# argumentcomputer/multi-stark

Measured on AMD Instinct MI355X. Metric: prove_trace_rows_per_sec, higher is better.
Workload: dtype u64; 1 GPU; U32-add + byte-table lookup (benches/multi_stark.rs), 2^20 additions per proof, bench_config(): log_blowup 2, 100 queries, 10+10 PoW bits, GoldilocksBlake3Config; witness (traces + claims, 64-bit words) in pinned host memory at step start: upload, from_stage_1 on the device and read-back inside the timed region; the library narrows byte-valued traces on host threads INSIDE the step before they cro; rows_per_proof=1048832, proof_bytes=1100053, parallelism=single GPU

## Files before the change

multi-stark_amd/csrc/lookup.hip:

```cpp
#include "lookup_params.h"
#include "msamd.h"
#include "program.h"

namespace msamd {

namespace {

constexpr int INV_CHUNK = 16;
constexpr int CLAIMS_CHUNK = 16;
__device__ __forceinline__ E2 message(const u64* __restrict__ a, u32 n, E2 beta, E2 gamma, const GammaPows& gp) {
  if (n <= gp.n) {
    GlAcc a0, a1;
    acc_init(a0);
    acc_init(a1);
    for (u32 k = 0; k < n; k++) {
      const u64 v = a[k];
      acc_mad(a0, v, gp.g[k].c0);
      acc_mad(a1, v, gp.g[k].c1);
    }
    return e2(gl_add(acc_reduce(a0), beta.c0), gl_add(acc_reduce(a1), beta.c1));
  }
  E2 f = e2(0);
  for (u32 k = n; k-- > 0;) {
    f = e2_mul(f, gamma);
// ... 110 lines not shown
    }
    E2 c = carry;
    if (i < nb) tot[i] = e2_add(c, e2_sub(sh[threadIdx.x], v));
    __syncthreads();
    if (threadIdx.x == 255) carry = e2_add(c, sh[255]);
    __syncthreads();
  }
  if (threadIdx.x == 0) *total = carry;
}
__global__ __launch_bounds__(256) void scan_add_k(E2* __restrict__ out, size_t n, const E2* __restrict__ block_prefix) {
  size_t base = (blockIdx.x * size_t(256) + threadIdx.x) * SCAN_ITEMS;
  E2 p = block_prefix[blockIdx.x];
#pragma unroll
  for (int k = 0; k < SCAN_ITEMS; k++)
    if (base + k < n) out[base + k] = e2_add(out[base + k], p);
}

__global__ __launch_bounds__(256) void claims_acc_k(const u64* __restrict__ data, const u64* __restrict__ offs, size_t n,
                                                    const ChallengeBG* __restrict__ ch, E2* __restrict__ partial) {
  __shared__ E2 sh[256];
  const E2 beta = ch->beta, gamma = ch->gamma;
  const GammaPows& gp = ch->gp;
  const size_t base = blockIdx.x * size_t(256 * CLAIMS_CHUNK) + threadIdx.x;
  E2 msg[CLAIMS_CHUNK];
  E2 sum = e2(0);
  int cnt = 0;
#pragma unroll
  for (int t = 0; t < CLAIMS_CHUNK; t++) {
    size_t i = base + size_t(t) * 256;
    if (i < n) {
// ... 84 lines not shown
  DBuf<E2> block_prefix;
  scan_exclusive(ctx, rowsum.p, prefix.p, n, total_dev, &block_prefix);
  ev = ctx.prof_begin(K_STAGE2);
  hipLaunchKernelGGL(stage2_write_k, grid, dim3(256), 0, ctx.stream, (const E2*)terms.p, n, logn, L, (const E2*)prefix.p, out,
                     (const E2*)block_prefix.p, SCAN_PER_BLOCK);
  ctx.prof_end(K_STAGE2, ev, double(n) * 16.0 * L);
  HIP_CHECK(hipGetLastError());
}

void stage2_from_trace_async(Ctx& ctx, const JitKernel& trace_jit, const u64* d_trace, const u64* d_pre, size_t n, size_t num_lookups,
                             size_t args_width, E2 beta, E2 gamma, u64* out, E2* total_dev) {
  DBuf<ChallengeBG> ch = challenge_bg_upload(ctx, beta, gamma);
  stage2_from_trace_dyn(ctx, trace_jit, d_trace, d_pre, n, num_lookups, args_width, ch.p, out, total_dev);
}
void stage2_from_trace_dyn(Ctx& ctx, const JitKernel& trace_jit, const u64* d_trace, const u64* d_pre, size_t n, size_t num_lookups,
                           size_t args_width, const ChallengeBG* ch, u64* out, E2* total_dev) {
  if (!trace_jit.function || num_lookups == 0) throw std::runtime_error("stage2_from_trace: no fused kernel for this circuit");
  const unsigned logn = log2_strict(n);
  const u32 L = (u32)num_lookups;
  DBuf<E2> rowsum(ctx, n), prefix(ctx, n), terms(ctx, n * L);
  dim3 grid((unsigned)((n + 255) / 256));
  Stage2TraceParams sp;
  sp.trace = d_trace;
  sp.pre = d_pre;
  sp.n = n;
  sp.ch = ch;
  sp.terms = terms.p;
  sp.rowsum = rowsum.p;
  hipEvent_t ev = ctx.prof_begin(K_STAGE2);
  stage2_trace_jit_launch(ctx, trace_jit, sp);
  ctx.prof_end(K_STAGE2, ev, double(n) * 8.0 * (L + args_width));
  DBuf<E2> block_prefix;
  scan_exclusive(ctx, rowsum.p, prefix.p, n, total_dev, &block_prefix);
  ev = ctx.prof_begin(K_STAGE2);
  hipLaunchKernelGGL(stage2_write_k, grid, dim3(256), 0, ctx.stream, (const E2*)terms.p, n, logn, L, (const E2*)prefix.p, out,
                     (const E2*)block_prefix.p, SCAN_PER_BLOCK);
  ctx.prof_end(K_STAGE2, ev, double(n) * 16.0 * L);
  HIP_CHECK(hipGetLastError());
}

E2 stage2_build(Ctx& ctx, const DLookups& lk, E2 beta, E2 gamma, u64* out, const JitKernel* jit) {
  DBuf<E2> tot(ctx, 1);
  stage2_build_async(ctx, lk, beta, gamma, out, tot.p, jit);
// ... 46 lines not shown
```

multi-stark_amd/csrc/lookup_params.h:

```cpp
#pragma once
#include "gl_dev.h"

namespace msamd {

constexpr int MAX_GPOW = 64;

struct GammaPows {
  E2 g[MAX_GPOW];
  u32 n;
};

struct ChallengeBG {
  E2 beta, gamma;
  GammaPows gp;
};
GL_HD void challenge_bg_fill(ChallengeBG& c, E2 beta, E2 gamma) {
  c.beta = beta;
  c.gamma = gamma;
  c.gp.n = MAX_GPOW;
  E2 g = e2(1);
  for (int i = 0; i < MAX_GPOW; i++) {
    c.gp.g[i] = g;
    g = e2_mul(g, gamma);
  }
// ... 3 lines not shown
  const u64* mult;
  const u64* args;
  size_t n;
  const ChallengeBG* ch;
  E2* terms;
  E2* rowsum;
};

struct Stage2TraceParams {
  const u64* trace;
  const u64* pre;
  size_t n;
  const ChallengeBG* ch;
  E2* terms;
  E2* rowsum;
};

}
```

multi-stark_amd/csrc/msamd.h:

```cpp
#pragma once
#include <hip/hip_runtime.h>

#include <cstdint>
#include <cstring>
#include <map>
#include <mutex>
#include <stdexcept>
#include <string>
#include <vector>

#include "gl_dev.h"

namespace msamd {

#define HIP_CHECK(expr)                                                                                   \
  do {                                                                                                    \
    hipError_t _e = (expr);                                                                               \
    if (_e != hipSuccess)                                                                                 \
      throw std::runtime_error(std::string("HIP error: ") + hipGetErrorString(_e) + " at " + __FILE__ + ":" + \
                               std::to_string(__LINE__));                                                 \
  } while (0)

static constexpr unsigned TW_LOG = 28;
static constexpr unsigned TW_HALF = 14;
// ... 172 lines not shown
  ~DBuf() { reset(); }
};

struct DMat {
  DBuf<u64> buf;
  size_t h = 0, w = 0;
  u64* d() const { return buf.p; }
};

struct NttSrc {
  const u64* src = nullptr;
  unsigned src_div = 1;
  const u64* scale = nullptr;
};
void ntt_dif(Ctx& ctx, u64* data, unsigned logn, size_t ncols, bool inverse, const NttSrc* from = nullptr, u64 out_mul = 1);
void ntt_dit(Ctx& ctx, u64* data, unsigned logn, size_t ncols, bool inverse, u64 out_mul = 1);
void transpose_in(Ctx& ctx, const u64* rowmajor, u64* colmajor, size_t h, size_t w, bool bitrev_rows);
void transpose_out(Ctx& ctx, const u64* colmajor, u64* rowmajor, size_t h, size_t w, bool bitrev_rows);
void pull_widen_words(const uint8_t* host_packed, unsigned bytes, size_t count, u64* out, hipStream_t stream);
void lde_from_coeffs(Ctx& ctx, const u64* coef, u64* lde, unsigned logn, unsigned log_blowup, size_t w);
void coset_lde(Ctx& ctx, u64* evals_bitrev, u64* lde, unsigned logn, unsigned log_blowup, size_t w);
void quotient_lde(Ctx& ctx, u64* qvals_bitrev, u64* lde, unsigned logn, unsigned logq, unsigned log_blowup, size_t D);

struct MatRef {
  const u64* d;
  uint32_t w;
  uint32_t pad;
  uint64_t stride;
};
struct DTree {
  std::vector<const u64*> mat_d;
  std::vector<size_t> mat_h, mat_w;
  std::vector<size_t> mat_stride;
  DBuf<Digest> digests;
  Digest* ext = nullptr;
  Digest* base() const { return ext ? ext : digests.p; }
// ... 34 lines not shown
                               u32* d_state12 = nullptr);

struct JitKernel;
struct DLookups {
  size_t height = 0, num_lookups = 0, args_width = 0;
  DBuf<u64> mult, args;
  DBuf<uint32_t> arg_offsets;
};
E2 stage2_build(Ctx& ctx, const DLookups& lk, E2 beta, E2 gamma, u64* out_colmajor_bitrev, const JitKernel* jit = nullptr);
void stage2_build_async(Ctx& ctx, const DLookups& lk, E2 beta, E2 gamma, u64* out_colmajor_bitrev, E2* total_dev,
                        const JitKernel* jit = nullptr);
struct ChallengeBG;
DBuf<ChallengeBG> challenge_bg_upload(Ctx& ctx, E2 beta, E2 gamma);
void stage2_build_dyn(Ctx& ctx, const DLookups& lk, const ChallengeBG* ch, u64* out_colmajor_bitrev, E2* total_dev, const JitKernel* jit = nullptr);
void stage2_from_trace_dyn(Ctx& ctx, const JitKernel& trace_jit, const u64* d_trace, const u64* d_pre, size_t n, size_t num_lookups,
                           size_t args_width, const ChallengeBG* ch, u64* out_colmajor_bitrev, E2* total_dev);
void claims_accumulator_dyn(Ctx& ctx, const u64* d_claim_data, const u64* d_claim_offsets, size_t n_claims, const ChallengeBG* ch, E2* out_dev);
void stage2_from_trace_async(Ctx& ctx, const JitKernel& trace_jit, const u64* d_trace, const u64* d_pre, size_t n, size_t num_lookups,
                             size_t args_width, E2 beta, E2 gamma, u64* out_colmajor_bitrev, E2* total_dev);
void claims_accumulator_async(Ctx& ctx, const u64* d_claim_data, const u64* d_claim_offsets, size_t n_claims, E2 beta, E2 gamma,
                              E2* out_dev);
E2 claims_accumulator(Ctx& ctx, const u64* d_claim_data, const u64* d_claim_offsets, size_t n_claims, E2 beta, E2 gamma);
size_t claims_transcript_words(Ctx& ctx, const u64* d_claim_data, const u64* d_claim_offsets, size_t n_claims,
                               size_t total_elems, u64* d_words);

void claims_transcript_words_slice(Ctx& ctx, const u64* d_data_abs, const u64* d_offs_first, size_t first, size_t count, size_t n_total,
                                   u64* d_words_abs);

struct JitKernel {
  void* module = nullptr;
  void* function = nullptr;
  bool inline_tables = false;
  unsigned groups = 0;
  JitKernel() {}
  JitKernel(const JitKernel&) = delete;
  JitKernel& operator=(const JitKernel&) = delete;
  JitKernel(JitKernel&& o) noexcept : module(o.module), function(o.function), inline_tables(o.inline_tables), groups(o.groups) {
    o.module = o.function = nullptr;
  }
  JitKernel& operator=(JitKernel&& o) noexcept {
    std::swap(module, o.module);
    std::swap(function, o.function);
    std::swap(inline_tables, o.inline_tables);
    std::swap(groups, o.groups);
    return *this;
  }
  ~JitKernel();
};
struct DProgram {
  JitKernel jit;
  DBuf<uint32_t> code;
  DBuf<u64> consts;
  size_t n_instr = 0, n_slots = 0;
  DBuf<uint32_t> zero_slots;
  DBuf<uint32_t> lookup_slots;
  size_t n_zeros = 0, n_lookups = 0, constraint_count = 0;
  size_t main_w = 0, pre_w = 0, s2_w = 0;
// ... 126 lines not shown
```

multi-stark_amd/csrc/ntt.hip:

```cpp
#include <cstring>

#include "msamd.h"

namespace msamd {

namespace {

__device__ __forceinline__ u64 tw_lookup(const u64* __restrict__ t0, const u64* __restrict__ t1, u32 e26) {
  return gl_mul(t1[e26 >> TW_HALF], t0[e26 & ((1u << TW_HALF) - 1)]);
}

template <int DIT>
__device__ __forceinline__ void lds_stages(u64* sm, unsigned k, unsigned logT, const u64* __restrict__ t1) {
  if (k == 0) return;
  const unsigned T = 1u << logT;
  const unsigned nb = (1u << (k - 1)) << logT;
  for (unsigned s = 0; s < k; s++) {
    const unsigned loghalf = DIT ? s : (k - 1 - s);
    const unsigned half = 1u << loghalf;
    const unsigned tsh = TW_HALF - loghalf - 1;
    for (unsigned b = threadIdx.x; b < nb; b += blockDim.x) {
      unsigned l = b & (T - 1), bb = b >> logT;
      unsigned j = bb & (half - 1), grp = bb >> loghalf;
      unsigned i0 = (((grp << (loghalf + 1)) + j) << logT) + l;
// ... 4 lines not shown
        u64 t = gl_mul(w, y);
        sm[i0] = gl_add(x, t);
        sm[i1] = gl_sub(x, t);
      } else {
        sm[i0] = gl_add(x, y);
        sm[i1] = gl_mul(gl_sub(x, y), w);
      }
    }
    __syncthreads();
  }
}

template <int DIT>
__global__ __launch_bounds__(256) void ntt_contig_k(const u64* __restrict__ src, u64* __restrict__ dst, unsigned K,
                                                     unsigned logn, const u64* __restrict__ t1, unsigned src_div,
                                                     const u64* __restrict__ scale, u64 out_mul) {
  extern __shared__ u64 sm[];
  const size_t n = size_t(1) << logn;
  const size_t col = blockIdx.y, off = size_t(blockIdx.x) << K;
  const u64* s = src + (col / src_div) * n + off;
  const u64* sc = scale ? scale + (col % src_div) * n + off : nullptr;
  u64* d = dst + col * n + off;
  const unsigned m = 1u << K;
  for (unsigned i = threadIdx.x; i < m; i += blockDim.x) {
    u64 v = s[i];
    if (sc) v = gl_mul(v, sc[i]);
    sm[i] = v;
  }
  __syncthreads();
  lds_stages<DIT>(sm, K, 0, t1);
  for (unsigned i = threadIdx.x; i < m; i += blockDim.x) {
    u64 v = sm[i];
    if (out_mul != 1) v = gl_mul(v, out_mul);
    d[i] = v;
  }
}

template <int DIT>
__global__ __launch_bounds__(256) void ntt_strided_k(const u64* __restrict__ src, u64* __restrict__ dst, unsigned k,
                                                      unsigned logS, unsigned logT, unsigned logn,
// ... 165 lines not shown
__device__ __forceinline__ void reg_round16(u64 (&x)[16], u32 lo, unsigned shift, const u64* __restrict__ twc, const u64* __restrict__ twx) {
#if MSAMD_R16TW
  (void)twc;
  reg_stages16_tw<DIT, INV>(x, lo, shift, twx);
#else
  reg_stages16_r4<DIT, INV>(x, lo, shift, twc, twx);
#endif
}

__device__ __forceinline__ u32 pad_hi(u32 e) { return e + ((e >> 8) << 4); }
__device__ __forceinline__ u32 pad_lo(u32 e) { return e + (e >> 4); }
constexpr int NTT12_LDS = 4096 + 256 + 16;
__device__ __forceinline__ u32 pad_half(u32 e) { return e + ((e >> 7) << 3); }
constexpr int NTT8S_LDS = 2048 + 128 + 8;

template <bool DIT, bool INV>
__global__ __launch_bounds__(256) void ntt12_k(const u64* __restrict__ src, u64* __restrict__ dst, unsigned logn,
                                               const u64* __restrict__ twc, const u64* __restrict__ twc3, unsigned src_div,
                                               const u64* __restrict__ scale, u64 out_mul) {
  __shared__ u64 sm[NTT12_LDS];
  const size_t n = size_t(1) << logn;
  const size_t col = blockIdx.y, off = size_t(blockIdx.x) << 12;
  const u64* s = src + (col / src_div) * n + off;
  const u64* sc = scale ? scale + (col % src_div) * n + off : nullptr;
  u64* d = dst + col * n + off;
  const u32 t = threadIdx.x, a = t >> 4, b = t & 15;
  u64 x[16];
#pragma unroll
  for (int j = 0; j < 16; j++) {
    u64 v = s[t + 256 * j];
    if (sc) v = gl_mul(v, sc[t + 256 * j]);
    x[j] = v;
  }
  if (!DIT) {
    reg_round16<false, INV>(x, t, 8, twc, twc3);
#pragma unroll
    for (int j = 0; j < 16; j++) sm[pad_hi(t + 256 * j)] = x[j];
    __syncthreads();
#pragma unroll
    for (int j = 0; j < 16; j++) x[j] = sm[pad_hi(a * 256 + 16 * j + b)];
    reg_round16<false, INV>(x, b, 4, twc, twc3);
    __syncthreads();
#pragma unroll
    for (int j = 0; j < 16; j++) sm[pad_lo(a * 256 + 16 * j + b)] = x[j];
    __syncthreads();
// ... 302 lines not shown
  unsigned logT = 12 - k;
  if (logT > logS) logT = logS;
  size_t gx = (size_t(1) << (logS - logT)) << (logn - logB);
  if (ncols > 65535) throw std::runtime_error("ntt: more than 65535 columns in one generic strided pass");
  dim3 grid((unsigned)gx, (unsigned)ncols);
  size_t shmem = (size_t(8) << (k + logT));
  hipEvent_t ev = ctx.prof_begin(K_NTT_STRIDED);
  hipLaunchKernelGGL(ntt_strided_k<DIT>, grid, dim3(256), shmem, ctx.stream, src, dst, k, logS, logT, logn,
                     inverse ? ctx.tw0i : ctx.tw0, inverse ? ctx.tw1i : ctx.tw1, src_div, scale, out_mul);
  HIP_CHECK(hipGetLastError());
  ctx.prof_end(K_NTT_STRIDED, ev, 16.0 * double(ncols) * double(size_t(1) << logn));
}

template <int DIT>
void launch_contig(Ctx& ctx, const u64* src, u64* dst, unsigned K, unsigned logn, size_t ncols, bool inverse,
                   unsigned src_div, const u64* scale, u64 out_mul) {
  dim3 grid((unsigned)(size_t(1) << (logn - K)), (unsigned)ncols);
  if (K == 12) {
    const int id = DIT ? K_NTT12_DIT : K_NTT12_DIF;
    hipEvent_t ev12 = ctx.prof_begin(id);
    if (inverse)
      hipLaunchKernelGGL((ntt12_k<(DIT != 0), true>), grid, dim3(256), 0, ctx.stream, src, dst, logn, ctx.twci, MSAMD_R16TW ? ctx.twfi : ctx.twc3i, src_div, scale, out_mul);
    else
      hipLaunchKernelGGL((ntt12_k<(DIT != 0), false>), grid, dim3(256), 0, ctx.stream, src, dst, logn, ctx.twc, MSAMD_R16TW ? ctx.twf : ctx.twc3, src_div, scale, out_mul);
    ctx.prof_end(id, ev12, 16.0 * double(ncols) * double(size_t(1) << logn));
    return;
  }
  unsigned threads = K >= 9 ? 256 : 64;
  hipEvent_t ev = ctx.prof_begin(K_NTT_CONTIG);
  hipLaunchKernelGGL(ntt_contig_k<DIT>, grid, dim3(threads), size_t(8) << K, ctx.stream, src, dst, K, logn,
                     inverse ? ctx.tw1i : ctx.tw1, src_div, scale, out_mul);
  ctx.prof_end(K_NTT_CONTIG, ev, 16.0 * double(ncols) * double(size_t(1) << logn));
}

void check_dims(unsigned logn, size_t ncols) {
  if (logn > NTT_MAX_LOG) throw std::runtime_error("ntt: transform larger than 2^26 is not supported");
  if (ncols > 65535) throw std::runtime_error("ntt: more than 65535 columns in one batch");
}

__global__ void lde_scale_k(u64* out, unsigned logn, unsigned lb) {
  size_t n = size_t(1) << logn;
  size_t i = blockIdx.x * size_t(blockDim.x) + threadIdx.x;
  if (i >= (n << lb)) return;
  size_t b = i >> logn, j = i & (n - 1);
  u64 wN = gl_two_adic_generator(logn + lb);
  u64 s = gl_mul(GL_GEN, gl_pow(wN, bitrev32((u32)b, lb)));
// ... 86 lines not shown
  Plan p = make_plan(logn);
  const u64* src = from && from->src ? from->src : data;
  unsigned src_div = from ? from->src_div : 1;
  const u64* scale = from ? from->scale : nullptr;
  unsigned logB = logn;
  for (size_t i = 0; i < p.bits.size(); i++) {
    launch_strided<0>(ctx, src, data, p.bits[i], logB, logn, ncols, inverse, src_div, scale, 1);
    src = data;
    src_div = 1;
    scale = nullptr;
    logB -= p.bits[i];
  }
  launch_contig<0>(ctx, src, data, p.K, logn, ncols, inverse, src_div, scale, out_mul);
}

void ntt_dit(Ctx& ctx, u64* data, unsigned logn, size_t ncols, bool inverse, u64 out_mul) {
  check_dims(logn, ncols);
  if (ncols == 0) return;
  Plan p = make_plan(logn);
  launch_contig<1>(ctx, data, data, p.K, logn, ncols, inverse, 1, nullptr, p.bits.empty() ? out_mul : 1);
  unsigned logB = p.K;
  for (size_t i = p.bits.size(); i-- > 0;) {
    logB += p.bits[i];
    launch_strided<1>(ctx, data, data, p.bits[i], logB, logn, ncols, inverse, 1, nullptr, i == 0 ? out_mul : 1);
  }
}

const u64* Ctx::lde_scale(unsigned log_n, unsigned log_blowup) {
  auto key = std::make_pair(log_n, log_blowup);
  auto it = lde_scales.find(key);
  if (it != lde_scales.end()) return it->second;
  size_t cnt = size_t(1) << (log_n + log_blowup);
  u64* p = nullptr;
  HIP_CHECK(hipMalloc(&p, cnt * 8));
  hipLaunchKernelGGL(lde_scale_k, dim3((unsigned)((cnt + 255) / 256)), dim3(256), 0, stream, p, log_n, log_blowup);
  HIP_CHECK(hipGetLastError());
  lde_scales[key] = p;
  return p;
}

void lde_from_coeffs(Ctx& ctx, const u64* coef, u64* lde, unsigned logn, unsigned log_blowup, size_t w) {
  NttSrc from;
  from.src = coef;
  from.src_div = 1u << log_blowup;
  from.scale = ctx.lde_scale(logn, log_blowup);
  ntt_dif(ctx, lde, logn, w << log_blowup, false, &from, 1);
}

void coset_lde(Ctx& ctx, u64* evals_bitrev, u64* lde, unsigned logn, unsigned log_blowup, size_t w) {
  ntt_dit(ctx, evals_bitrev, logn, w, true, 1);
  lde_from_coeffs(ctx, evals_bitrev, lde, logn, log_blowup, w);
}

void quotient_lde(Ctx& ctx, u64* qvals_bitrev, u64* lde, unsigned logn, unsigned logq, unsigned log_blowup, size_t D) {
  unsigned logN = logn + logq;
  ntt_dit(ctx, qvals_bitrev, logN, D, false, 1);
  size_t q = size_t(1) << logq, n = size_t(1) << logn;
  std::vector<u64> wk(q);
  u64 n_inv = gl_inv((u64)(n << logq));
  u64 step = gl_inv(gl_pow(GL_GEN, (u64)n)), cur = 1;
  for (size_t k = 0; k < q; k++) {
    wk[k] = gl_mul(cur, n_inv);
    cur = gl_mul(cur, step);
  }
  WkTab tab;
// ... 87 lines not shown
```

multi-stark_amd/csrc/program.h:

```cpp
#pragma once
#include <cstdint>
#include <utility>
#include <vector>

#include "msamd.h"

namespace msamd {

enum : uint32_t { OP_CONST = 0, OP_VAR, OP_PUBLIC, OP_IS_FIRST, OP_IS_LAST, OP_IS_TRANS, OP_ADD, OP_SUB, OP_MUL, OP_NEG };

struct PNode {
  uint32_t kind = 0, source = 0, offset = 0;
  uint64_t a = 0, b = 0;
};

void build_program(Ctx& ctx, const std::vector<PNode>& nodes, const std::vector<uint32_t>& zeros,
                   const std::vector<std::pair<uint32_t, std::vector<uint32_t>>>& lookups, DProgram& out);

struct QParams;
void quotient_jit_build(const std::vector<PNode>& nodes, const std::vector<uint32_t>& zeros,
                        const std::vector<std::pair<uint32_t, std::vector<uint32_t>>>& lookups, size_t quotient_degree, JitKernel& out);
void quotient_jit_launch(Ctx& ctx, const JitKernel& k, const QParams& p, size_t nq);
void bb_quotient_jit_build(const std::vector<PNode>& nodes, const std::vector<uint32_t>& zeros,
                           const std::vector<std::pair<uint32_t, std::vector<uint32_t>>>& lookups, JitKernel& out);
void bb_quotient_jit_launch(Ctx& ctx, const JitKernel& k, const void* args, size_t args_size, size_t rows);
struct Stage2Params;
struct Stage2TraceParams;
void stage2_jit_build(const std::vector<uint32_t>& arg_counts, JitKernel& out);
void stage2_jit_launch(Ctx& ctx, const JitKernel& k, const Stage2Params& p);
void stage2_trace_jit_build(const std::vector<PNode>& nodes, const std::vector<std::pair<uint32_t, std::vector<uint32_t>>>& lookups,
                            size_t main_w, size_t pre_w, size_t prefix_len, JitKernel& out);
void stage2_trace_jit_launch(Ctx& ctx, const JitKernel& k, const Stage2TraceParams& p);

bool lookup_values_device(Ctx& ctx, const DProgram& prefix, const u64* d_trace, const u64* d_pre, size_t h, size_t main_w,
                          size_t pre_w, size_t args_w, u64* d_mult, u64* d_args, hipStream_t on_stream = nullptr);

}
```

multi-stark_amd/csrc/prover.hip:

```cpp
#include <algorithm>
#include <chrono>
#include <cstdio>
#include <cstdlib>

#include <sys/resource.h>
#include <unistd.h>

#include <atomic>
#include <condition_variable>
#include <functional>
#include <mutex>
#include <thread>

#include "host.h"
#include "ingest.h"
#include "lookup_params.h"
#include "open_plan.h"
#include "quotient_params.h"

namespace msamd {

namespace {
void load_block(const uint8_t* p, size_t len, u32 w[16]) {
  uint8_t buf[64];
// ... 1724 lines not shown
      index_i >>= la;
      size_t ns = n_siblings(trees[i]);
      w.u64_(ns);
      w.raw(&g[pos], ns * 32);
      pos += ns * 32;
    }
  }
  w.u64_(final_poly.size());
  for (auto& e : final_poly) w.ext(e);
  w.u64_(query_pow);
  g_probes.mark("FriProof bytes written");
  if (host_trace) fprintf(stderr, "[msamd] host work after the FRI read-back: %.1f us (transcript replay + FriProof bytes)\n", 1e3 * (now_ms() - t_sync));
}
}

void stage2_circuit_dyn(Ctx& ctx, const HSystem& sys, const HWitness& wit, size_t ci, const ChallengeBG* bg, u64* out, E2* total_dev) {
  const HCircuit& c = sys.circuits[ci];
  const DLookups& lk = wit.lookups[ci];
  if (c.num_lookups && !lk.mult.p) {
    if (!c.stage2_trace_jit.function || !wit.traces[ci].p) throw std::runtime_error("stage 2: this circuit has neither lookup values nor a fused kernel");
    stage2_from_trace_dyn(ctx, c.stage2_trace_jit, wit.traces[ci].p, c.pre_width ? c.d_preprocessed.p : nullptr, wit.heights[ci], c.num_lookups,
                          c.args_width, bg, out, total_dev);
    return;
  }
  stage2_build_dyn(ctx, lk, bg, out, total_dev, &c.stage2_jit);
}
void stage2_circuit_async(Ctx& ctx, const HSystem& sys, const HWitness& wit, size_t ci, E2 beta, E2 gamma, u64* out, E2* total_dev) {
  DBuf<ChallengeBG> bg = challenge_bg_upload(ctx, beta, gamma);
  stage2_circuit_dyn(ctx, sys, wit, ci, bg.p, out, total_dev);
}

void observe_claims(Ctx& ctx, Challenger& ch, HWitness& wit) {
  const size_t n_claims = wit.claim_offsets.size() - 1;
  const size_t claim_elems = wit.claim_data.size();
  const size_t claim_words = 1 + n_claims + claim_elems;
  if (claim_words <= 8192) {
    ch.observe((u64)n_claims);
// ... 206 lines not shown
    if (!claims_beside) claims_sum_launch();
  } else {
    E2 acc0 = e2(0);
    for (size_t i = 0; i < n_claims; i++) {
      E2 f = e2(0);
      for (size_t k = wit.claim_offsets[i + 1]; k-- > wit.claim_offsets[i];) f = e2_add(e2_mul(f, gamma), e2(wit.claim_data[k]));
      acc0 = e2_add(acc0, e2_inv(e2_add(beta, f)));
    }
    ctx.h2d(d_tot.p, &acc0, sizeof(E2));
  }

  t0 = now_ms();
  phase.next("stark/lookup_construction");
  up.lookup_values();
  std::vector<DBuf<u64>> s2_evals(NA);
  fork_side();
  for (size_t pos : order) {
    size_t ci = aidx[pos];
    const HCircuit& c = sys.circuits[ci];
    size_t n = wit.heights[ci];
    SideScope sc(ctx, on_side[pos]);
    s2_evals[pos] = DBuf<u64>(ctx, n * c.stage2_width);
    stage2_circuit_dyn(ctx, sys, wit, ci, d_bg.p, s2_evals[pos].p, d_tot.p + 1 + pos);
  }
  if (claims_beside) claims_sum_launch();
  lap(1);
  t0 = now_ms();
  phase.next("stark/stage2_commit");
  PcsData s2;
  {
    std::vector<DMat> ldes(NA);
    fork_side();
    for (size_t pos : order) {
      const HCircuit& c = sys.circuits[aidx[pos]];
      size_t n = wit.heights[aidx[pos]];
      SideScope sc(ctx, on_side[pos]);
      DMat lde;
      lde.h = n << lb;
      lde.w = c.stage2_width;
      lde.buf = DBuf<u64>(ctx, lde.h * lde.w);
      coset_lde(ctx, s2_evals[pos].p, lde.d(), log_degrees[pos], lb, lde.w);
      s2_evals[pos].reset();
      ldes[pos] = std::move(lde);
    }
    ctx.side_join();
    commit_matrices(ctx, std::move(ldes), (unsigned)prm.cap_height, s2);
  }
  ctx.d2h_queue(h_tot.data(), d_tot.p, (NA + 1) * sizeof(E2));
  g_probes.mark("stage 2 queued");
  auto dev_cap = [&](const DTree& t) -> const Digest* {
    const size_t cl = t.cap_layer();
    if (t.layer_len[cl] != ncap) throw std::runtime_error("a commitment's cap size differs from the stage-1 cap");
    return t.base() + t.layer_off[cl];
  };
  std::vector<Digest> s2_cap, q_cap;
  E2 acc_initial = e2(0);
  std::vector<E2> accs;
// ... 193 lines not shown
```

multi-stark_amd/csrc/quotient_jit.hip:

```cpp
#include <dlfcn.h>
#include <sys/stat.h>
#include <unistd.h>

#include <cstdio>
#include <cstdlib>
#include <map>
#include <mutex>
#include <sstream>

#include "bb_dev.h"
#include "host.h"
#include "lookup_params.h"
#include "quotient_params.h"

namespace msamd {

namespace {

bool inline_tables_fit(size_t n_zeros, size_t n_lookups, size_t quotient_degree) {
  return n_zeros + 2 * std::max<size_t>(n_lookups, 1) <= QP_INLINE_ALPHA && quotient_degree <= 8;
}

std::string circuit_source(const std::vector<PNode>& nodes, const std::vector<uint32_t>& zeros,
                           const std::vector<std::pair<uint32_t, std::vector<uint32_t>>>& lookups, bool inl) {
// ... 475 lines not shown
    needed[l.first] = 1;
    for (auto a : l.second) needed[a] = 1;
  }
  for (size_t i = nn; i-- > 0;) {
    if (!needed[i]) continue;
    const PNode& n = nodes[i];
    if (n.kind == OP_ADD || n.kind == OP_SUB || n.kind == OP_MUL) needed[n.a] = needed[n.b] = 1;
    if (n.kind == OP_NEG) needed[n.a] = 1;
  }
  std::vector<char> used[2][2];
  for (int s2 = 0; s2 < 2; s2++)
    for (int of = 0; of < 2; of++) used[s2][of].assign(s2 ? main_w : pre_w, 0);
  for (size_t i = 0; i < nn; i++)
    if (needed[i] && nodes[i].kind == OP_VAR) used[nodes[i].source][nodes[i].offset][nodes[i].a] = 1;
  std::ostringstream o;
  o << "#include \"lookup_params.h\"\nusing namespace msamd;\n"
       "extern \"C\" __global__ __launch_bounds__(256) void stage2_terms_trace_jit(Stage2TraceParams p) {\n"
       "  const size_t r = blockIdx.x * size_t(blockDim.x) + threadIdx.x;\n"
       "  if (r >= p.n) return;\n"
       "  const size_t rn = r + 1 == p.n ? 0 : r + 1;\n"
       "  const u64 is_first = r == 0, is_last = r + 1 == p.n, is_trans = r + 1 != p.n;\n"
       "  (void)is_first; (void)is_last; (void)is_trans; (void)rn;\n";
  for (int s2 = 0; s2 < 2; s2++)
    for (int of = 0; of < 2; of++) {
      const size_t W = s2 ? main_w : pre_w;
      const char* base = s2 ? "p.trace" : "p.pre";
      const std::string nm = std::string(s2 ? "m" : "q") + (of ? "n" : "c");
      bool any = false;
      for (char u : used[s2][of]) any = any || u;
      if (!any) continue;
      o << "  const u64* __restrict__ " << nm << " = " << base << " + " << (of ? "rn" : "r") << " * " << W << ";\n";
      if (W % 2 == 0) {
        for (size_t k = 0; k < W; k += 2)
          if (used[s2][of][k] || used[s2][of][k + 1])
            o << "  const ulonglong2 " << nm << "p" << k << " = reinterpret_cast<const ulonglong2*>(" << nm << ")[" << k / 2 << "]; const u64 "
              << nm << k << " = " << nm << "p" << k << ".x, " << nm << k + 1 << " = " << nm << "p" << k << ".y; (void)" << nm << k << "; (void)"
              << nm << k + 1 << ";\n";
      } else {
        for (size_t k = 0; k < W; k++)
          if (used[s2][of][k]) o << "  const u64 " << nm << k << " = " << nm << "[" << k << "];\n";
      }
    }
  for (size_t i = 0; i < nn; i++) {
    if (!needed[i]) continue;
    const PNode& n = nodes[i];
    o << "  const u64 v" << i << " = ";
    switch (n.kind) {
      case OP_CONST: o << n.a << "ULL"; break;
      case OP_VAR: o << (n.source ? "m" : "q") << (n.offset ? "n" : "c") << n.a; break;
      case OP_IS_FIRST: o << "is_first"; break;
      case OP_IS_LAST: o << "is_last"; break;
      case OP_IS_TRANS: o << "is_trans"; break;
      case OP_ADD: o << "gl_add(v" << n.a << ", v" << n.b << ")"; break;
      case OP_SUB: o << "gl_sub(v" << n.a << ", v" << n.b << ")"; break;
      case OP_MUL: o << "gl_mul(v" << n.a << ", v" << n.b << ")"; break;
      case OP_NEG: o << "gl_neg(v" << n.a << ")"; break;
      default: o << "0ULL"; break;
    }
    o << ";\n";
  }
  o << "  E2 s = e2(0);\n  E2* __restrict__ trow = p.terms + r * " << L << ";\n";
  for (size_t j0 = 0; j0 < L; j0 += 16) {
    const size_t cnt = std::min<size_t>(16, L - j0);
    o << "  {\n    E2 msg[16];\n";
    for (size_t t = 0; t < cnt; t++) {
      const auto& l = lookups[j0 + t];
      o << "    { GlAcc g0, g1; acc_init(g0); acc_init(g1);\n";
      for (size_t k = 0; k < l.second.size(); k++)
        o << "      acc_mad(g0, v" << l.second[k] << ", p.ch->gp.g[" << k << "].c0); acc_mad(g1, v" << l.second[k] << ", p.ch->gp.g[" << k << "].c1);\n";
      o << "      msg[" << t << "] = e2(gl_add(acc_reduce(g0), p.ch->beta.c0), gl_add(acc_reduce(g1), p.ch->beta.c1)); }\n";
    }
    o << "    e2_batch_inverse<16>(msg, " << cnt << ");\n";
    for (size_t t = 0; t < cnt; t++) {
      const size_t j = j0 + t;
      o << "    { const E2 v = e2_mul_base(msg[" << t << "], v" << lookups[j].first << "); trow[" << j << "] = v; s = e2_add(s, v); }\n";
    }
    o << "  }\n";
  }
  o << "  p.rowsum[r] = s;\n}\n";
  return o.str();
}
}

void quotient_jit_build(const std::vector<PNode>& nodes, const std::vector<uint32_t>& zeros,
                        const std::vector<std::pair<uint32_t, std::vector<uint32_t>>>& lookups, size_t quotient_degree, JitKernel& out) {
  if (getenv("MSAMD_NO_JIT")) return;
  if (nodes.size() > 3000) return;
  const bool inl = inline_tables_fit(zeros.size(), lookups.size(), quotient_degree);
  load_kernel(code_object(circuit_source(nodes, zeros, lookups, inl)), "quotient_jit", out);
  out.inline_tables = out.function && inl;
}

void bb_quotient_jit_build(const std::vector<PNode>& nodes, const std::vector<uint32_t>& zeros,
                           const std::vector<std::pair<uint32_t, std::vector<uint32_t>>>& lookups, JitKernel& out) {
// ... 21 lines not shown
  out.groups = out.function ? G : 0u;
}

void stage2_trace_jit_build(const std::vector<PNode>& nodes, const std::vector<std::pair<uint32_t, std::vector<uint32_t>>>& lookups,
                            size_t main_w, size_t pre_w, size_t prefix_len, JitKernel& out) {
  if (getenv("MSAMD_NO_JIT") || getenv("MSAMD_NO_STAGE2_FUSION") || lookups.empty() || lookups.size() > 256 || prefix_len > 3000) return;
  size_t aw = 0;
  for (auto& l : lookups) {
    if (l.second.size() > (size_t)MAX_GPOW) return;
    aw += l.second.size();
  }
  if (aw > 1024) return;
  for (size_t i = 0; i < prefix_len; i++)
    if (nodes[i].kind == OP_PUBLIC || (nodes[i].kind == OP_VAR && nodes[i].source == 2)) return;
  load_kernel(code_object(stage2_trace_source(nodes, lookups, main_w, pre_w)), "stage2_terms_trace_jit", out);
}

void stage2_trace_jit_launch(Ctx& ctx, const JitKernel& k, const Stage2TraceParams& p) {
  Stage2TraceParams copy = p;
  size_t size = sizeof(Stage2TraceParams);
  void* config[] = {HIP_LAUNCH_PARAM_BUFFER_POINTER, &copy, HIP_LAUNCH_PARAM_BUFFER_SIZE, &size, HIP_LAUNCH_PARAM_END};
  HIP_CHECK(hipModuleLaunchKernel((hipFunction_t)k.function, (unsigned)((p.n + 255) / 256), 1, 1, 256, 1, 1, 0, ctx.stream, nullptr, config));
}

void stage2_jit_launch(Ctx& ctx, const JitKernel& k, const Stage2Params& p) {
  Stage2Params copy = p;
  size_t size = sizeof(Stage2Params);
  void* config[] = {HIP_LAUNCH_PARAM_BUFFER_POINTER, &copy, HIP_LAUNCH_PARAM_BUFFER_SIZE, &size, HIP_LAUNCH_PARAM_END};
  if (k.groups)
    HIP_CHECK(hipModuleLaunchKernel((hipFunction_t)k.function, (unsigned)((p.n + 63) / 64), 1, 1, 64 * k.groups, 1, 1, 0, ctx.stream, nullptr, config));
  else
    HIP_CHECK(hipModuleLaunchKernel((hipFunction_t)k.function, (unsigned)((p.n + 255) / 256), 1, 1, 256, 1, 1, 0, ctx.stream, nullptr, config));
}

void quotient_jit_launch(Ctx& ctx, const JitKernel& k, const QParams& p, size_t nq) {
  QParams copy = p;
  size_t size = sizeof(QParams);
// ... 6 lines not shown
```

Measured before the change: 162.6 million rows/s.

## Write stage-2 columns directly and fold the row prefix into the inverse NTT

```diff
diff --git a/multi-stark_amd/csrc/lookup.hip b/multi-stark_amd/csrc/lookup.hip
--- a/multi-stark_amd/csrc/lookup.hip
+++ b/multi-stark_amd/csrc/lookup.hip
@@ -148,6 +148,15 @@
 #pragma unroll
   for (int k = 0; k < SCAN_ITEMS; k++)
     if (base + k < n) out[base + k] = e2_add(out[base + k], p);
+}
+
+__global__ __launch_bounds__(256) void scan_row_add_k(const E2* __restrict__ rowprefix, const E2* __restrict__ block_prefix, u32 per,
+                                                      unsigned logn, u64* __restrict__ row_add) {
+  size_t r, rr;
+  stage2_tile_rows(blockIdx.x, threadIdx.x, logn, r, rr);
+  const E2 v = e2_add(rowprefix[r], block_prefix[r / per]);
+  row_add[rr] = v.c0;
+  row_add[(size_t(1) << logn) + rr] = v.c1;
 }
 
 __global__ __launch_bounds__(256) void claims_acc_k(const u64* __restrict__ data, const u64* __restrict__ offs, size_t n,
@@ -262,10 +271,34 @@
   stage2_from_trace_dyn(ctx, trace_jit, d_trace, d_pre, n, num_lookups, args_width, ch.p, out, total_dev);
 }
 void stage2_from_trace_dyn(Ctx& ctx, const JitKernel& trace_jit, const u64* d_trace, const u64* d_pre, size_t n, size_t num_lookups,
-                           size_t args_width, const ChallengeBG* ch, u64* out, E2* total_dev) {
+                           size_t args_width, const ChallengeBG* ch, u64* out, E2* total_dev, DBuf<u64>* row_add_out) {
   if (!trace_jit.function || num_lookups == 0) throw std::runtime_error("stage2_from_trace: no fused kernel for this circuit");
   const unsigned logn = log2_strict(n);
   const u32 L = (u32)num_lookups;
+  if (row_add_out) row_add_out->reset();
+  if (row_add_out && trace_jit.function_cols && n >= 256 && (size_t(1) << logn) == n) {
+    DBuf<E2> rowsum(ctx, n), prefix(ctx, n);
+    DBuf<u64> row_add(ctx, 2 * n);
+    Stage2TraceParams sp;
+    sp.trace = d_trace;
+    sp.pre = d_pre;
+    sp.n = n;
+    sp.ch = ch;
+    sp.terms = nullptr;
+    sp.rowsum = rowsum.p;
+    sp.cols = out;
+    sp.logn = logn;
+    hipEvent_t ev = ctx.prof_begin(K_STAGE2);
+    stage2_cols_trace_jit_launch(ctx, trace_jit, sp);
+    ctx.prof_end(K_STAGE2, ev, double(n) * 8.0 * (2.0 * L + args_width));
+    DBuf<E2> block_prefix;
+    scan_exclusive(ctx, rowsum.p, prefix.p, n, total_dev, &block_prefix);
+    hipLaunchKernelGGL(scan_row_add_k, dim3((unsigned)(n >> 8)), dim3(256), 0, ctx.stream, (const E2*)prefix.p, (const E2*)block_prefix.p,
+                       SCAN_PER_BLOCK, logn, row_add.p);
+    HIP_CHECK(hipGetLastError());
+    *row_add_out = std::move(row_add);
+    return;
+  }
   DBuf<E2> rowsum(ctx, n), prefix(ctx, n), terms(ctx, n * L);
   dim3 grid((unsigned)((n + 255) / 256));
   Stage2TraceParams sp;
@@ -275,6 +308,8 @@
   sp.ch = ch;
   sp.terms = terms.p;
   sp.rowsum = rowsum.p;
+  sp.cols = nullptr;
+  sp.logn = logn;
   hipEvent_t ev = ctx.prof_begin(K_STAGE2);
   stage2_trace_jit_launch(ctx, trace_jit, sp);
   ctx.prof_end(K_STAGE2, ev, double(n) * 8.0 * (L + args_width));
diff --git a/multi-stark_amd/csrc/lookup_params.h b/multi-stark_amd/csrc/lookup_params.h
--- a/multi-stark_amd/csrc/lookup_params.h
+++ b/multi-stark_amd/csrc/lookup_params.h
@@ -4,6 +4,7 @@
 namespace msamd {
 
 constexpr int MAX_GPOW = 64;
+constexpr int STAGE2_COLS_MAX_LOOKUPS = 32;
 
 struct GammaPows {
   E2 g[MAX_GPOW];
@@ -41,6 +42,14 @@
   const ChallengeBG* ch;
   E2* terms;
   E2* rowsum;
+  u64* cols;
+  u32 logn;
 };
 
+__device__ __forceinline__ void stage2_tile_rows(u32 mid, u32 t, u32 logn, size_t& r, size_t& rr) {
+  const u32 u = t & 15, a = t >> 4;
+  r = (size_t(u) << (logn - 4)) | (size_t(bitrev32(mid, logn - 8)) << 4) | a;
+  rr = (size_t(bitrev32(a, 4)) << (logn - 4)) | (size_t(mid) << 4) | bitrev32(u, 4);
 }
+
+}
diff --git a/multi-stark_amd/csrc/msamd.h b/multi-stark_amd/csrc/msamd.h
--- a/multi-stark_amd/csrc/msamd.h
+++ b/multi-stark_amd/csrc/msamd.h
@@ -210,12 +210,12 @@
   const u64* scale = nullptr;
 };
 void ntt_dif(Ctx& ctx, u64* data, unsigned logn, size_t ncols, bool inverse, const NttSrc* from = nullptr, u64 out_mul = 1);
-void ntt_dit(Ctx& ctx, u64* data, unsigned logn, size_t ncols, bool inverse, u64 out_mul = 1);
+void ntt_dit(Ctx& ctx, u64* data, unsigned logn, size_t ncols, bool inverse, u64 out_mul = 1, const u64* row_add = nullptr);
 void transpose_in(Ctx& ctx, const u64* rowmajor, u64* colmajor, size_t h, size_t w, bool bitrev_rows);
 void transpose_out(Ctx& ctx, const u64* colmajor, u64* rowmajor, size_t h, size_t w, bool bitrev_rows);
 void pull_widen_words(const uint8_t* host_packed, unsigned bytes, size_t count, u64* out, hipStream_t stream);
 void lde_from_coeffs(Ctx& ctx, const u64* coef, u64* lde, unsigned logn, unsigned log_blowup, size_t w);
-void coset_lde(Ctx& ctx, u64* evals_bitrev, u64* lde, unsigned logn, unsigned log_blowup, size_t w);
+void coset_lde(Ctx& ctx, u64* evals_bitrev, u64* lde, unsigned logn, unsigned log_blowup, size_t w, const u64* row_add = nullptr);
 void quotient_lde(Ctx& ctx, u64* qvals_bitrev, u64* lde, unsigned logn, unsigned logq, unsigned log_blowup, size_t D);
 
 struct MatRef {
@@ -280,7 +280,8 @@
 DBuf<ChallengeBG> challenge_bg_upload(Ctx& ctx, E2 beta, E2 gamma);
 void stage2_build_dyn(Ctx& ctx, const DLookups& lk, const ChallengeBG* ch, u64* out_colmajor_bitrev, E2* total_dev, const JitKernel* jit = nullptr);
 void stage2_from_trace_dyn(Ctx& ctx, const JitKernel& trace_jit, const u64* d_trace, const u64* d_pre, size_t n, size_t num_lookups,
-                           size_t args_width, const ChallengeBG* ch, u64* out_colmajor_bitrev, E2* total_dev);
+                           size_t args_width, const ChallengeBG* ch, u64* out_colmajor_bitrev, E2* total_dev,
+                           DBuf<u64>* row_add_out = nullptr);
 void claims_accumulator_dyn(Ctx& ctx, const u64* d_claim_data, const u64* d_claim_offsets, size_t n_claims, const ChallengeBG* ch, E2* out_dev);
 void stage2_from_trace_async(Ctx& ctx, const JitKernel& trace_jit, const u64* d_trace, const u64* d_pre, size_t n, size_t num_lookups,
                              size_t args_width, E2 beta, E2 gamma, u64* out_colmajor_bitrev, E2* total_dev);
@@ -298,15 +299,18 @@
   void* function = nullptr;
   bool inline_tables = false;
   unsigned groups = 0;
+  void* function_cols = nullptr;
   JitKernel() {}
   JitKernel(const JitKernel&) = delete;
   JitKernel& operator=(const JitKernel&) = delete;
-  JitKernel(JitKernel&& o) noexcept : module(o.module), function(o.function), inline_tables(o.inline_tables), groups(o.groups) {
-    o.module = o.function = nullptr;
+  JitKernel(JitKernel&& o) noexcept
+      : module(o.module), function(o.function), inline_tables(o.inline_tables), groups(o.groups), function_cols(o.function_cols) {
+    o.module = o.function = o.function_cols = nullptr;
   }
   JitKernel& operator=(JitKernel&& o) noexcept {
     std::swap(module, o.module);
     std::swap(function, o.function);
+    std::swap(function_cols, o.function_cols);
     std::swap(inline_tables, o.inline_tables);
     std::swap(groups, o.groups);
     return *this;
diff --git a/multi-stark_amd/csrc/ntt.hip b/multi-stark_amd/csrc/ntt.hip
--- a/multi-stark_amd/csrc/ntt.hip
+++ b/multi-stark_amd/csrc/ntt.hip
@@ -42,16 +42,18 @@
 template <int DIT>
 __global__ __launch_bounds__(256) void ntt_contig_k(const u64* __restrict__ src, u64* __restrict__ dst, unsigned K,
                                                      unsigned logn, const u64* __restrict__ t1, unsigned src_div,
-                                                     const u64* __restrict__ scale, u64 out_mul) {
+                                                     const u64* __restrict__ scale, u64 out_mul, const u64* __restrict__ row_add) {
   extern __shared__ u64 sm[];
   const size_t n = size_t(1) << logn;
   const size_t col = blockIdx.y, off = size_t(blockIdx.x) << K;
   const u64* s = src + (col / src_div) * n + off;
   const u64* sc = scale ? scale + (col % src_div) * n + off : nullptr;
+  const u64* ra = row_add ? row_add + (col & 1) * n + off : nullptr;
   u64* d = dst + col * n + off;
   const unsigned m = 1u << K;
   for (unsigned i = threadIdx.x; i < m; i += blockDim.x) {
     u64 v = s[i];
+    if (ra) v = gl_add(v, ra[i]);
     if (sc) v = gl_mul(v, sc[i]);
     sm[i] = v;
   }
@@ -247,21 +249,23 @@
 __device__ __forceinline__ u32 pad_half(u32 e) { return e + ((e >> 7) << 3); }
 constexpr int NTT8S_LDS = 2048 + 128 + 8;
 
-template <bool DIT, bool INV>
+template <bool DIT, bool INV, bool RADD = false>
 __global__ __launch_bounds__(256) void ntt12_k(const u64* __restrict__ src, u64* __restrict__ dst, unsigned logn,
                                                const u64* __restrict__ twc, const u64* __restrict__ twc3, unsigned src_div,
-                                               const u64* __restrict__ scale, u64 out_mul) {
+                                               const u64* __restrict__ scale, u64 out_mul, const u64* __restrict__ row_add) {
   __shared__ u64 sm[NTT12_LDS];
   const size_t n = size_t(1) << logn;
   const size_t col = blockIdx.y, off = size_t(blockIdx.x) << 12;
   const u64* s = src + (col / src_div) * n + off;
   const u64* sc = scale ? scale + (col % src_div) * n + off : nullptr;
+  const u64* ra = RADD ? row_add + (col & 1) * n + off : nullptr;
   u64* d = dst + col * n + off;
   const u32 t = threadIdx.x, a = t >> 4, b = t & 15;
   u64 x[16];
 #pragma unroll
   for (int j = 0; j < 16; j++) {
     u64 v = s[t + 256 * j];
+    if (RADD) v = gl_add(v, ra[t + 256 * j]);
     if (sc) v = gl_mul(v, sc[t + 256 * j]);
     x[j] = v;
   }
@@ -594,22 +598,26 @@
 
 template <int DIT>
 void launch_contig(Ctx& ctx, const u64* src, u64* dst, unsigned K, unsigned logn, size_t ncols, bool inverse,
-                   unsigned src_div, const u64* scale, u64 out_mul) {
+                   unsigned src_div, const u64* scale, u64 out_mul, const u64* row_add = nullptr) {
   dim3 grid((unsigned)(size_t(1) << (logn - K)), (unsigned)ncols);
+  if (row_add && !(DIT && inverse && src_div == 1)) throw std::runtime_error("ntt: a row addend goes with the first pass of an inverse ntt_dit only");
   if (K == 12) {
     const int id = DIT ? K_NTT12_DIT : K_NTT12_DIF;
     hipEvent_t ev12 = ctx.prof_begin(id);
-    if (inverse)
-      hipLaunchKernelGGL((ntt12_k<(DIT != 0), true>), grid, dim3(256), 0, ctx.stream, src, dst, logn, ctx.twci, MSAMD_R16TW ? ctx.twfi : ctx.twc3i, src_div, scale, out_mul);
+    const u64* no_add = nullptr;
+    if (row_add)
+      hipLaunchKernelGGL((ntt12_k<true, true, true>), grid, dim3(256), 0, ctx.stream, src, dst, logn, ctx.twci, MSAMD_R16TW ? ctx.twfi : ctx.twc3i, src_div, scale, out_mul, row_add);
+    else if (inverse)
+      hipLaunchKernelGGL((ntt12_k<(DIT != 0), true>), grid, dim3(256), 0, ctx.stream, src, dst, logn, ctx.twci, MSAMD_R16TW ? ctx.twfi : ctx.twc3i, src_div, scale, out_mul, no_add);
     else
-      hipLaunchKernelGGL((ntt12_k<(DIT != 0), false>), grid, dim3(256), 0, ctx.stream, src, dst, logn, ctx.twc, MSAMD_R16TW ? ctx.twf : ctx.twc3, src_div, scale, out_mul);
+      hipLaunchKernelGGL((ntt12_k<(DIT != 0), false>), grid, dim3(256), 0, ctx.stream, src, dst, logn, ctx.twc, MSAMD_R16TW ? ctx.twf : ctx.twc3, src_div, scale, out_mul, no_add);
     ctx.prof_end(id, ev12, 16.0 * double(ncols) * double(size_t(1) << logn));
     return;
   }
   unsigned threads = K >= 9 ? 256 : 64;
   hipEvent_t ev = ctx.prof_begin(K_NTT_CONTIG);
   hipLaunchKernelGGL(ntt_contig_k<DIT>, grid, dim3(threads), size_t(8) << K, ctx.stream, src, dst, K, logn,
-                     inverse ? ctx.tw1i : ctx.tw1, src_div, scale, out_mul);
+                     inverse ? ctx.tw1i : ctx.tw1, src_div, scale, out_mul, row_add);
   ctx.prof_end(K_NTT_CONTIG, ev, 16.0 * double(ncols) * double(size_t(1) << logn));
 }
 
@@ -726,11 +734,11 @@
   launch_contig<0>(ctx, src, data, p.K, logn, ncols, inverse, src_div, scale, out_mul);
 }
 
-void ntt_dit(Ctx& ctx, u64* data, unsigned logn, size_t ncols, bool inverse, u64 out_mul) {
+void ntt_dit(Ctx& ctx, u64* data, unsigned logn, size_t ncols, bool inverse, u64 out_mul, const u64* row_add) {
   check_dims(logn, ncols);
   if (ncols == 0) return;
   Plan p = make_plan(logn);
-  launch_contig<1>(ctx, data, data, p.K, logn, ncols, inverse, 1, nullptr, p.bits.empty() ? out_mul : 1);
+  launch_contig<1>(ctx, data, data, p.K, logn, ncols, inverse, 1, nullptr, p.bits.empty() ? out_mul : 1, row_add);
   unsigned logB = p.K;
   for (size_t i = p.bits.size(); i-- > 0;) {
     logB += p.bits[i];
@@ -759,8 +767,8 @@
   ntt_dif(ctx, lde, logn, w << log_blowup, false, &from, 1);
 }
 
-void coset_lde(Ctx& ctx, u64* evals_bitrev, u64* lde, unsigned logn, unsigned log_blowup, size_t w) {
-  ntt_dit(ctx, evals_bitrev, logn, w, true, 1);
+void coset_lde(Ctx& ctx, u64* evals_bitrev, u64* lde, unsigned logn, unsigned log_blowup, size_t w, const u64* row_add) {
+  ntt_dit(ctx, evals_bitrev, logn, w, true, 1, row_add);
   lde_from_coeffs(ctx, evals_bitrev, lde, logn, log_blowup, w);
 }
 
diff --git a/multi-stark_amd/csrc/program.h b/multi-stark_amd/csrc/program.h
--- a/multi-stark_amd/csrc/program.h
+++ b/multi-stark_amd/csrc/program.h
@@ -31,6 +31,7 @@
 void stage2_trace_jit_build(const std::vector<PNode>& nodes, const std::vector<std::pair<uint32_t, std::vector<uint32_t>>>& lookups,
                             size_t main_w, size_t pre_w, size_t prefix_len, JitKernel& out);
 void stage2_trace_jit_launch(Ctx& ctx, const JitKernel& k, const Stage2TraceParams& p);
+void stage2_cols_trace_jit_launch(Ctx& ctx, const JitKernel& k, const Stage2TraceParams& p);
 
 bool lookup_values_device(Ctx& ctx, const DProgram& prefix, const u64* d_trace, const u64* d_pre, size_t h, size_t main_w,
                           size_t pre_w, size_t args_w, u64* d_mult, u64* d_args, hipStream_t on_stream = nullptr);
diff --git a/multi-stark_amd/csrc/prover.hip b/multi-stark_amd/csrc/prover.hip
--- a/multi-stark_amd/csrc/prover.hip
+++ b/multi-stark_amd/csrc/prover.hip
@@ -1762,13 +1762,15 @@
 }
 }
 
-void stage2_circuit_dyn(Ctx& ctx, const HSystem& sys, const HWitness& wit, size_t ci, const ChallengeBG* bg, u64* out, E2* total_dev) {
+void stage2_circuit_dyn(Ctx& ctx, const HSystem& sys, const HWitness& wit, size_t ci, const ChallengeBG* bg, u64* out, E2* total_dev,
+                        DBuf<u64>* row_add = nullptr) {
+  if (row_add) row_add->reset();
   const HCircuit& c = sys.circuits[ci];
   const DLookups& lk = wit.lookups[ci];
   if (c.num_lookups && !lk.mult.p) {
     if (!c.stage2_trace_jit.function || !wit.traces[ci].p) throw std::runtime_error("stage 2: this circuit has neither lookup values nor a fused kernel");
     stage2_from_trace_dyn(ctx, c.stage2_trace_jit, wit.traces[ci].p, c.pre_width ? c.d_preprocessed.p : nullptr, wit.heights[ci], c.num_lookups,
-                          c.args_width, bg, out, total_dev);
+                          c.args_width, bg, out, total_dev, row_add);
     return;
   }
   stage2_build_dyn(ctx, lk, bg, out, total_dev, &c.stage2_jit);
@@ -2005,6 +2007,8 @@
   phase.next("stark/lookup_construction");
   up.lookup_values();
   std::vector<DBuf<u64>> s2_evals(NA);
+  std::vector<DBuf<u64>> s2_row_add(NA);
+  const bool s2_two_pass = getenv("MSAMD_STAGE2_TWO_PASS") != nullptr;
   fork_side();
   for (size_t pos : order) {
     size_t ci = aidx[pos];
@@ -2012,7 +2016,7 @@
     size_t n = wit.heights[ci];
     SideScope sc(ctx, on_side[pos]);
     s2_evals[pos] = DBuf<u64>(ctx, n * c.stage2_width);
-    stage2_circuit_dyn(ctx, sys, wit, ci, d_bg.p, s2_evals[pos].p, d_tot.p + 1 + pos);
+    stage2_circuit_dyn(ctx, sys, wit, ci, d_bg.p, s2_evals[pos].p, d_tot.p + 1 + pos, s2_two_pass ? nullptr : &s2_row_add[pos]);
   }
   if (claims_beside) claims_sum_launch();
   lap(1);
@@ -2030,8 +2034,9 @@
       lde.h = n << lb;
       lde.w = c.stage2_width;
       lde.buf = DBuf<u64>(ctx, lde.h * lde.w);
-      coset_lde(ctx, s2_evals[pos].p, lde.d(), log_degrees[pos], lb, lde.w);
+      coset_lde(ctx, s2_evals[pos].p, lde.d(), log_degrees[pos], lb, lde.w, s2_row_add[pos].p);
       s2_evals[pos].reset();
+      s2_row_add[pos].reset();
       ldes[pos] = std::move(lde);
     }
     ctx.side_join();
diff --git a/multi-stark_amd/csrc/quotient_jit.hip b/multi-stark_amd/csrc/quotient_jit.hip
--- a/multi-stark_amd/csrc/quotient_jit.hip
+++ b/multi-stark_amd/csrc/quotient_jit.hip
@@ -513,70 +513,86 @@
   for (size_t i = 0; i < nn; i++)
     if (needed[i] && nodes[i].kind == OP_VAR) used[nodes[i].source][nodes[i].offset][nodes[i].a] = 1;
   std::ostringstream o;
-  o << "#include \"lookup_params.h\"\nusing namespace msamd;\n"
-       "extern \"C\" __global__ __launch_bounds__(256) void stage2_terms_trace_jit(Stage2TraceParams p) {\n"
-       "  const size_t r = blockIdx.x * size_t(blockDim.x) + threadIdx.x;\n"
-       "  if (r >= p.n) return;\n"
-       "  const size_t rn = r + 1 == p.n ? 0 : r + 1;\n"
-       "  const u64 is_first = r == 0, is_last = r + 1 == p.n, is_trans = r + 1 != p.n;\n"
-       "  (void)is_first; (void)is_last; (void)is_trans; (void)rn;\n";
-  for (int s2 = 0; s2 < 2; s2++)
-    for (int of = 0; of < 2; of++) {
-      const size_t W = s2 ? main_w : pre_w;
-      const char* base = s2 ? "p.trace" : "p.pre";
-      const std::string nm = std::string(s2 ? "m" : "q") + (of ? "n" : "c");
-      bool any = false;
-      for (char u : used[s2][of]) any = any || u;
-      if (!any) continue;
-      o << "  const u64* __restrict__ " << nm << " = " << base << " + " << (of ? "rn" : "r") << " * " << W << ";\n";
-      if (W % 2 == 0) {
-        for (size_t k = 0; k < W; k += 2)
-          if (used[s2][of][k] || used[s2][of][k + 1])
-            o << "  const ulonglong2 " << nm << "p" << k << " = reinterpret_cast<const ulonglong2*>(" << nm << ")[" << k / 2 << "]; const u64 "
-              << nm << k << " = " << nm << "p" << k << ".x, " << nm << k + 1 << " = " << nm << "p" << k << ".y; (void)" << nm << k << "; (void)"
-              << nm << k + 1 << ";\n";
-      } else {
-        for (size_t k = 0; k < W; k++)
-          if (used[s2][of][k]) o << "  const u64 " << nm << k << " = " << nm << "[" << k << "];\n";
+  o << "#include \"lookup_params.h\"\nusing namespace msamd;\n";
+  auto emit = [&](bool cols) {
+    if (cols)
+      o << "extern \"C\" __global__ __launch_bounds__(256) void stage2_cols_trace_jit(Stage2TraceParams p) {\n"
+           "  size_t r, rr;\n"
+           "  stage2_tile_rows(blockIdx.x, threadIdx.x, p.logn, r, rr);\n"
+           "  u64* __restrict__ col = p.cols + rr;\n";
+    else
+      o << "extern \"C\" __global__ __launch_bounds__(256) void stage2_terms_trace_jit(Stage2TraceParams p) {\n"
+           "  const size_t r = blockIdx.x * size_t(blockDim.x) + threadIdx.x;\n"
+           "  if (r >= p.n) return;\n";
+    o << "  const size_t rn = r + 1 == p.n ? 0 : r + 1;\n"
+         "  const u64 is_first = r == 0, is_last = r + 1 == p.n, is_trans = r + 1 != p.n;\n"
+         "  (void)is_first; (void)is_last; (void)is_trans; (void)rn;\n";
+    for (int s2 = 0; s2 < 2; s2++)
+      for (int of = 0; of < 2; of++) {
+        const size_t W = s2 ? main_w : pre_w;
+        const char* base = s2 ? "p.trace" : "p.pre";
+        const std::string nm = std::string(s2 ? "m" : "q") + (of ? "n" : "c");
+        bool any = false;
+        for (char u : used[s2][of]) any = any || u;
+        if (!any) continue;
+        o << "  const u64* __restrict__ " << nm << " = " << base << " + " << (of ? "rn" : "r") << " * " << W << ";\n";
+        if (W % 2 == 0) {
+          for (size_t k = 0; k < W; k += 2)
+            if (used[s2][of][k] || used[s2][of][k + 1])
+              o << "  const ulonglong2 " << nm << "p" << k << " = reinterpret_cast<const ulonglong2*>(" << nm << ")[" << k / 2 << "]; const u64 "
+                << nm << k << " = " << nm << "p" << k << ".x, " << nm << k + 1 << " = " << nm << "p" << k << ".y; (void)" << nm << k << "; (void)"
+                << nm << k + 1 << ";\n";
+        } else {
+          for (size_t k = 0; k < W; k++)
+            if (used[s2][of][k]) o << "  const u64 " << nm << k << " = " << nm << "[" << k << "];\n";
+        }
       }
-    }
-  for (size_t i = 0; i < nn; i++) {
-    if (!needed[i]) continue;
-    const PNode& n = nodes[i];
-    o << "  const u64 v" << i << " = ";
-    switch (n.kind) {
-      case OP_CONST: o << n.a << "ULL"; break;
-      case OP_VAR: o << (n.source ? "m" : "q") << (n.offset ? "n" : "c") << n.a; break;
-      case OP_IS_FIRST: o << "is_first"; break;
-      case OP_IS_LAST: o << "is_last"; break;
-      case OP_IS_TRANS: o << "is_trans"; break;
-      case OP_ADD: o << "gl_add(v" << n.a << ", v" << n.b << ")"; break;
-      case OP_SUB: o << "gl_sub(v" << n.a << ", v" << n.b << ")"; break;
-      case OP_MUL: o << "gl_mul(v" << n.a << ", v" << n.b << ")"; break;
-      case OP_NEG: o << "gl_neg(v" << n.a << ")"; break;
-      default: o << "0ULL"; break;
-    }
-    o << ";\n";
-  }
-  o << "  E2 s = e2(0);\n  E2* __restrict__ trow = p.terms + r * " << L << ";\n";
-  for (size_t j0 = 0; j0 < L; j0 += 16) {
-    const size_t cnt = std::min<size_t>(16, L - j0);
-    o << "  {\n    E2 msg[16];\n";
-    for (size_t t = 0; t < cnt; t++) {
-      const auto& l = lookups[j0 + t];
-      o << "    { GlAcc g0, g1; acc_init(g0); acc_init(g1);\n";
-      for (size_t k = 0; k < l.second.size(); k++)
-        o << "      acc_mad(g0, v" << l.second[k] << ", p.ch->gp.g[" << k << "].c0); acc_mad(g1, v" << l.second[k] << ", p.ch->gp.g[" << k << "].c1);\n";
-      o << "      msg[" << t << "] = e2(gl_add(acc_reduce(g0), p.ch->beta.c0), gl_add(acc_reduce(g1), p.ch->beta.c1)); }\n";
-    }
-    o << "    e2_batch_inverse<16>(msg, " << cnt << ");\n";
-    for (size_t t = 0; t < cnt; t++) {
-      const size_t j = j0 + t;
-      o << "    { const E2 v = e2_mul_base(msg[" << t << "], v" << lookups[j].first << "); trow[" << j << "] = v; s = e2_add(s, v); }\n";
-    }
-    o << "  }\n";
-  }
-  o << "  p.rowsum[r] = s;\n}\n";
+    for (size_t i = 0; i < nn; i++) {
+      if (!needed[i]) continue;
+      const PNode& n = nodes[i];
+      o << "  const u64 v" << i << " = ";
+      switch (n.kind) {
+        case OP_CONST: o << n.a << "ULL"; break;
+        case OP_VAR: o << (n.source ? "m" : "q") << (n.offset ? "n" : "c") << n.a; break;
+        case OP_IS_FIRST: o << "is_first"; break;
+        case OP_IS_LAST: o << "is_last"; break;
+        case OP_IS_TRANS: o << "is_trans"; break;
+        case OP_ADD: o << "gl_add(v" << n.a << ", v" << n.b << ")"; break;
+        case OP_SUB: o << "gl_sub(v" << n.a << ", v" << n.b << ")"; break;
+        case OP_MUL: o << "gl_mul(v" << n.a << ", v" << n.b << ")"; break;
+        case OP_NEG: o << "gl_neg(v" << n.a << ")"; break;
+        default: o << "0ULL"; break;
+      }
+      o << ";\n";
+    }
+    o << "  E2 s = e2(0);\n";
+    if (!cols) o << "  E2* __restrict__ trow = p.terms + r * " << L << ";\n";
+    for (size_t j0 = 0; j0 < L; j0 += 16) {
+      const size_t cnt = std::min<size_t>(16, L - j0);
+      o << "  {\n    E2 msg[16];\n";
+      for (size_t t = 0; t < cnt; t++) {
+        const auto& l = lookups[j0 + t];
+        o << "    { GlAcc g0, g1; acc_init(g0); acc_init(g1);\n";
+        for (size_t k = 0; k < l.second.size(); k++)
+          o << "      acc_mad(g0, v" << l.second[k] << ", p.ch->gp.g[" << k << "].c0); acc_mad(g1, v" << l.second[k] << ", p.ch->gp.g[" << k << "].c1);\n";
+        o << "      msg[" << t << "] = e2(gl_add(acc_reduce(g0), p.ch->beta.c0), gl_add(acc_reduce(g1), p.ch->beta.c1)); }\n";
+      }
+      o << "    e2_batch_inverse<16>(msg, " << cnt << ");\n";
+      for (size_t t = 0; t < cnt; t++) {
+        const size_t j = j0 + t;
+        o << "    { const E2 v = e2_mul_base(msg[" << t << "], v" << lookups[j].first << "); ";
+        if (cols)
+          o << "col[" << 2 * j << " * p.n] = s.c0; col[" << 2 * j + 1 << " * p.n] = s.c1;";
+        else
+          o << "trow[" << j << "] = v;";
+        o << " s = e2_add(s, v); }\n";
+      }
+      o << "  }\n";
+    }
+    o << "  p.rowsum[r] = s;\n}\n";
+  };
+  emit(false);
+  if (L <= STAGE2_COLS_MAX_LOOKUPS) emit(true);
   return o.str();
 }
 }
@@ -628,6 +644,11 @@
   for (size_t i = 0; i < prefix_len; i++)
     if (nodes[i].kind == OP_PUBLIC || (nodes[i].kind == OP_VAR && nodes[i].source == 2)) return;
   load_kernel(code_object(stage2_trace_source(nodes, lookups, main_w, pre_w)), "stage2_terms_trace_jit", out);
+  if (out.function && lookups.size() <= (size_t)STAGE2_COLS_MAX_LOOKUPS) {
+    hipFunction_t fn = nullptr;
+    if (hipModuleGetFunction(&fn, (hipModule_t)out.module, "stage2_cols_trace_jit") != hipSuccess) throw std::runtime_error("stage2_cols_trace_jit is missing from its module");
+    out.function_cols = fn;
+  }
 }
 
 void stage2_trace_jit_launch(Ctx& ctx, const JitKernel& k, const Stage2TraceParams& p) {
@@ -635,6 +656,14 @@
   size_t size = sizeof(Stage2TraceParams);
   void* config[] = {HIP_LAUNCH_PARAM_BUFFER_POINTER, &copy, HIP_LAUNCH_PARAM_BUFFER_SIZE, &size, HIP_LAUNCH_PARAM_END};
   HIP_CHECK(hipModuleLaunchKernel((hipFunction_t)k.function, (unsigned)((p.n + 255) / 256), 1, 1, 256, 1, 1, 0, ctx.stream, nullptr, config));
+}
+
+void stage2_cols_trace_jit_launch(Ctx& ctx, const JitKernel& k, const Stage2TraceParams& p) {
+  if (!k.function_cols || p.n < 256 || (size_t(1) << p.logn) != p.n) throw std::runtime_error("stage 2: the single-write kernel needs whole 256-row tiles");
+  Stage2TraceParams copy = p;
+  size_t size = sizeof(Stage2TraceParams);
+  void* config[] = {HIP_LAUNCH_PARAM_BUFFER_POINTER, &copy, HIP_LAUNCH_PARAM_BUFFER_SIZE, &size, HIP_LAUNCH_PARAM_END};
+  HIP_CHECK(hipModuleLaunchKernel((hipFunction_t)k.function_cols, (unsigned)(p.n >> 8), 1, 1, 256, 1, 1, 0, ctx.stream, nullptr, config));
 }
 
 void stage2_jit_launch(Ctx& ctx, const JitKernel& k, const Stage2Params& p) {
```

New measurement: 167.3 million rows/s, median of 5. 1.03x the previous value.
